# citibeth/spsparse

Hardware: AMD Instinct MI355X
Metric: nnz(C)/s for C=A*A SpGEMM (higher is better)
Workload: dtype f64

## Files before the change

### spsparse_amd/build.py

```python
import os
import subprocess
import sys
from concurrent.futures import ThreadPoolExecutor

HERE = os.path.dirname(os.path.abspath(__file__))
CSRC = os.path.join(HERE, "csrc")
VARIANT = os.environ.get("SPSAMD_VARIANT", "")
LIBDIR = os.path.join(HERE, "lib", VARIANT) if VARIANT else os.path.join(HERE, "lib")
LIB = os.path.join(LIBDIR, "libspsparse_amd.so")
SOURCES = ["prims.hip", "operand.hip", "sink.hip", "consolidate.hip", "spgemm.hip", "symbolic_heavy.hip", "k_light.hip", "k_hash.hip", "k_dense.hip", "k_tiles.hip", "k_spmm.hip", "k_add.hip", "k_stream.hip", "k_masked.hip", "k_sampled.hip", "k_select.hip", "k_extract.hip", "k_reduce.hip", "k_emult.hip", "k_solve.hip", "k_factor.hip", "k_color.hip", "k_aggregate.hip", "k_krylov.hip", "k_amg.hip",
           "workload.hip", "capi.hip", "dist.hip"]
HEADERS = ["internal.h", "devutil.h", "bank_layout.h", "spgemm_dev.h", "spgemm_host.h", "spgemm_hash.h", "workload_common.h", "x86fp.h", os.path.join("..", "..", "include", "spsparse_amd.h")]
FLAGS = ["--offload-arch=gfx950", "-O3", "-std=c++17", "-fPIC", "-ffp-contract=off",
         "-munsafe-fp-atomics", "-Wall", "-Wno-unused-result"]
FLAGS += os.environ.get("SPSAMD_CXXFLAGS", "").split()


def hipcc():
    for cand in (os.environ.get("HIPCC"), "/opt/rocm/bin/hipcc", "hipcc"):
        if cand and (os.path.isabs(cand) and os.path.exists(cand) or not os.path.isabs(cand)):
            return cand
    return "hipcc"


def _stale(target, deps):
    if not os.path.exists(target):
        return True
    t = os.path.getmtime(target)
    return any(os.path.getmtime(d) > t for d in deps)


def build(force=False, verbose=False):
    os.makedirs(LIBDIR, exist_ok=True)
    hdrs = [os.path.join(CSRC, h) for h in HEADERS]
    objs, jobs = [], []
    for s in SOURCES:
        src = os.path.join(CSRC, s)
        obj = os.path.join(LIBDIR, s.replace(".hip", ".o"))
        objs.append(obj)
        if force or _stale(obj, [src] + hdrs):
            jobs.append([hipcc()] + FLAGS + ["-c", src, "-o", obj])

    def run(cmd):
# ... 14 lines not shown
```

### spsparse_amd/csrc/capi.hip

```cpp
#include "internal.h"

#include <cstdio>
#include <cstdlib>
#include <cstring>
#include <algorithm>
#include <exception>
#include <vector>

using namespace spsamd;

#define API_GUARD(ctx, ...)                                                         \
	if ((ctx)->busy) { (ctx)->last_error = "context busy: a streamed multiply is delivering on it"; return SPSAMD_EINVAL; } \
	try { __VA_ARGS__ }                                                             \
	catch (const spsamd::Error &e) { (ctx)->last_error = e.msg; return e.code; }    \
	catch (const std::bad_alloc &) { (ctx)->last_error = "host allocation failed"; return SPSAMD_ENOMEM; } \
	catch (const std::exception &e) { (ctx)->last_error = e.what(); return SPSAMD_EINVAL; }

extern "C" const char *spsamd_version(void) { return "spsparse_amd 0.2 (gfx950)"; }

extern "C" int spsamd_ctx_create(spsamd_ctx **out, int device, void *hip_stream)
{
	if (!out) return SPSAMD_EINVAL;
	*out = nullptr;
	int ndev = 0;
	if (hipGetDeviceCount(&ndev) != hipSuccess || ndev == 0) { (void)hipGetLastError(); return SPSAMD_ENODEVICE; }
	if (device < 0) { if (hipGetDevice(&device) != hipSuccess) return SPSAMD_ENODEVICE; }
	if (device >= ndev) return SPSAMD_ENODEVICE;
	if (hipSetDevice(device) != hipSuccess) return SPSAMD_ENODEVICE;
	spsamd_ctx *c = new (std::nothrow) spsamd_ctx();
	if (!c) return SPSAMD_ENOMEM;
	c->device = device;
	hipDeviceProp_t prop;
	if (hipGetDeviceProperties(&prop, device) == hipSuccess) c->num_cu = prop.multiProcessorCount;
	if (hip_stream) { c->stream = (hipStream_t)hip_stream; c->own_stream = false; }
	else {
		if (hipStreamCreateWithFlags(&c->stream, hipStreamNonBlocking) != hipSuccess) { delete c; return SPSAMD_EHIP; }
		c->own_stream = true;
	}
	for (auto &e : c->ev) if (hipEventCreate(&e) != hipSuccess) { spsamd_ctx_destroy(c); return SPSAMD_EHIP; }
	for (auto &e : c->ev2) if (hipEventCreate(&e) != hipSuccess) { spsamd_ctx_destroy(c); return SPSAMD_EHIP; }
	if (hipStreamCreateWithFlags(&c->side, hipStreamNonBlocking) != hipSuccess) { spsamd_ctx_destroy(c); return SPSAMD_EHIP; }
	for (auto &e : c->ev_side) if (hipEventCreateWithFlags(&e, hipEventDisableTiming) != hipSuccess) { spsamd_ctx_destroy(c); return SPSAMD_EHIP; }
	if (hipStreamCreateWithFlags(&c->side2, hipStreamNonBlocking) != hipSuccess) { spsamd_ctx_destroy(c); return SPSAMD_EHIP; }
	for (auto &e : c->ev_side2) if (hipEventCreateWithFlags(&e, hipEventDisableTiming) != hipSuccess) { spsamd_ctx_destroy(c); return SPSAMD_EHIP; }
	static const char *const knobs[] = {"window", "cell_cap", "dense_min", "no_tiles", "xcd", "emit_path", "light_path", "no_wmajor", "direct_min", "tiles_v1", "long_cap", "long_dense_min", "index_budget_mb", "trace", "light_two_pass", "spmm_path", "spmm_long_min", "add_path", "masked_path", "sampled_path", "select_path", "extract_path", "reduce_path", "emult_path", "tile_walk", "solve_path", "solve_row", "solve_fuse_rows", "factor_path", "factor_row", "factor_fuse_rows", "factor_serial_work", "factor_lds_row", "color_path", "color_row", "color_fuse_rows", "color_wave_deg", "agg_path", "agg_row", "agg_fuse_rows", "agg_wave_deg", "agg_per_rows", "pcg_check_every", "pcg_fuse", "amg_path", "amg_fuse_rows"};
	static const char *const envs[] = {"SPSAMD_W", "SPSAMD_CELL_CAP", "SPSAMD_DENSE_MIN", "SPSAMD_NO_TILES", "SPSAMD_XCD", "SPSAMD_EMIT_PATH", "SPSAMD_LIGHT_PATH", "SPSAMD_NO_WMAJOR", "SPSAMD_DIRECT_MIN", "SPSAMD_TILES_V1", "SPSAMD_LONG_CAP", "SPSAMD_LONG_DENSE_MIN", "SPSAMD_INDEX_BUDGET_MB", "SPSAMD_TRACE", "SPSAMD_LIGHT_TWO_PASS", "SPSAMD_SPMM_PATH", "SPSAMD_SPMM_LONG_MIN", "SPSAMD_ADD_PATH", "SPSAMD_MASKED_PATH", "SPSAMD_SAMPLED_PATH", "SPSAMD_SELECT_PATH", "SPSAMD_EXTRACT_PATH", "SPSAMD_REDUCE_PATH", "SPSAMD_EMULT_PATH", "SPSAMD_TILE_WALK", "SPSAMD_SOLVE_PATH", "SPSAMD_SOLVE_ROW", "SPSAMD_SOLVE_FUSE_ROWS", "SPSAMD_FACTOR_PATH", "SPSAMD_FACTOR_ROW", "SPSAMD_FACTOR_FUSE_ROWS", "SPSAMD_FACTOR_SERIAL_WORK", "SPSAMD_FACTOR_LDS_ROW", "SPSAMD_COLOR_PATH", "SPSAMD_COLOR_ROW", "SPSAMD_COLOR_FUSE_ROWS", "SPSAMD_COLOR_WAVE_DEG", "SPSAMD_AGG_PATH", "SPSAMD_AGG_ROW", "SPSAMD_AGG_FUSE_ROWS", "SPSAMD_AGG_WAVE_DEG", "SPSAMD_AGG_PER_ROWS", "SPSAMD_PCG_CHECK_EVERY", "SPSAMD_PCG_FUSE", "SPSAMD_AMG_PATH", "SPSAMD_AMG_FUSE_ROWS"};
	static_assert(sizeof knobs / sizeof knobs[0] == sizeof envs / sizeof envs[0], "one environment variable per knob");
	for (size_t k = 0; k < sizeof knobs / sizeof knobs[0]; ++k)
		if (const char *e = getenv(envs[k])) (void)spsamd_ctx_set_tuning(c, knobs[k], atol(e));
#ifdef SPSAMD_ABLATIONS
	if (const char *e = getenv("SPSAMD_DBG")) c->tune.dbg = atoi(e);
#endif
	*out = c;
	return SPSAMD_OK;
}

extern "C" int spsamd_ctx_set_tuning(spsamd_ctx *c, const char *name, long value)
{
	if (!c || !name) return SPSAMD_EINVAL;
	if (c->busy) { c->last_error = "context busy: a streamed multiply is delivering on it"; return SPSAMD_EINVAL; }
	struct { const char *n; int *p; } tab[] = {
		{"window", &c->tune.window}, {"cell_cap", &c->tune.cell_cap}, {"dense_min", &c->tune.dense_min},
		{"no_tiles", &c->tune.no_tiles}, {"xcd", &c->tune.xcd}, {"emit_path", &c->tune.emit_path},
		{"light_path", &c->tune.light_path}, {"no_wmajor", &c->tune.no_wmajor}, {"direct_min", &c->tune.direct_min}, {"tiles_v1", &c->tune.tiles_v1}, {"long_cap", &c->tune.long_cap}, {"long_dense_min", &c->tune.long_dense_min}, {"index_budget_mb", &c->tune.index_budget_mb}, {"trace", &c->tune.trace}, {"light_two_pass", &c->tune.light_two_pass},
		{"spmm_path", &c->tune.spmm_path}, {"spmm_long_min", &c->tune.spmm_long_min}, {"add_path", &c->tune.add_path},
		{"masked_path", &c->tune.masked_path}, {"sampled_path", &c->tune.sampled_path}, {"select_path", &c->tune.select_path},
		{"extract_path", &c->tune.extract_path}, {"reduce_path", &c->tune.reduce_path}, {"emult_path", &c->tune.emult_path},
		{"tile_walk", &c->tune.tile_walk}, {"solve_path", &c->tune.solve_path}, {"solve_row", &c->tune.solve_row},
		{"solve_fuse_rows", &c->tune.solve_fuse_rows}, {"factor_path", &c->tune.factor_path}, {"factor_row", &c->tune.factor_row},
		{"factor_fuse_rows", &c->tune.factor_fuse_rows}, {"factor_serial_work", &c->tune.factor_serial_work},
		{"factor_lds_row", &c->tune.factor_lds_row}, {"color_path", &c->tune.color_path}, {"color_row", &c->tune.color_row},
		{"color_fuse_rows", &c->tune.color_fuse_rows}, {"color_wave_deg", &c->tune.color_wave_deg},
		{"agg_path", &c->tune.agg_path}, {"agg_row", &c->tune.agg_row}, {"agg_fuse_rows", &c->tune.agg_fuse_rows},
		{"agg_wave_deg", &c->tune.agg_wave_deg}, {"agg_per_rows", &c->tune.agg_per_rows},
		{"pcg_check_every", &c->tune.pcg_check_every}, {"pcg_fuse", &c->tune.pcg_fuse},
		{"amg_path", &c->tune.amg_path}, {"amg_fuse_rows", &c->tune.amg_fuse_rows},
	};
	for (auto &t : tab) if (!std::strcmp(t.n, name)) { *t.p = (int)value; return SPSAMD_OK; }
	c->last_error = std::string("unknown tuning knob: ") + name;
	return SPSAMD_EINVAL;
}

extern "C" void spsamd_ctx_destroy(spsamd_ctx *c)
{
	if (!c) return;
	(void)hipSetDevice(c->device);
	if (c->stream) (void)hipStreamSynchronize(c->stream);
	if (c->side) (void)hipStreamSynchronize(c->side);
	if (c->side2) (void)hipStreamSynchronize(c->side2);
	c->arena.release();
	c->out[0].release(); c->out[1].release();
	c->rowstat_n.release(); c->rowstat_s.release(); c->rowstat_h.release();
	if (c->pinned) (void)hipHostFree(c->pinned);
	if (c->stream_pinned) (void)hipHostFree(c->stream_pinned);
	for (auto &e : c->ev) if (e) (void)hipEventDestroy(e);
	for (auto &e : c->ev2) if (e) (void)hipEventDestroy(e);
	for (auto &e : c->ev_side) if (e) (void)hipEventDestroy(e);
// ... 573 lines not shown
```

### spsparse_amd/csrc/internal.h

```cpp
#pragma once

#include <hip/hip_runtime.h>
#include <stdint.h>
#include <stddef.h>
#include <string>
#include <vector>

#include "../../include/spsparse_amd.h"

namespace spsamd {


struct Error {
	int code;
	std::string msg;
};

#define SPS_HIP(call)                                                              \
	do {                                                                           \
		hipError_t e_ = (call);                                                    \
		if (e_ != hipSuccess)                                                      \
			throw ::spsamd::Error{SPSAMD_EHIP, std::string(#call) + ": " + hipGetErrorString(e_)}; \
	} while (0)

// ... 13 lines not shown
	void reset();
	void release();
	void reserve(size_t bytes);
	template <class T> T *get(size_t n) { return (T *)alloc(n * sizeof(T)); }
};

struct DevBuf {
	void *p = nullptr;
	size_t cap = 0;
	void ensure(size_t bytes);
	void release();
	bool holds(const void *q) const { return p && q && (const char *)q >= (const char *)p && (const char *)q < (const char *)p + cap; }
};

struct OutSet {
	DevBuf i, j, v;
	bool holds(const void *q) const { return i.holds(q) || j.holds(q) || v.holds(q); }
	void release() { i.release(); j.release(); v.release(); }
};

struct Tuning {
	int window = 0;
	int cell_cap = 0;
	int dense_min = 0;
	int no_tiles = 0;
	int xcd = 2;
	int emit_path = 0;
	int light_path = 0;
	int light_two_pass = 0;
	int no_wmajor = 0;
	int tiles_v1 = 0;
	int long_cap = 0;
	int long_dense_min = 0;
	int direct_min = 0;
	int trace = 0;
	int index_budget_mb = 0;
	int spmm_path = 0;
	int spmm_long_min = 0;
	int add_path = 0;
	int masked_path = 0;
	int sampled_path = 0;
	int select_path = 0;
	int extract_path = 0;
	int reduce_path = 0;
	int tile_walk = 0;
	int emult_path = 0;
	int solve_path = 0;
	int solve_row = 0;
	int solve_fuse_rows = 0;
	int factor_path = 0;
	int factor_row = 0;
	int factor_fuse_rows = 0;
	int factor_serial_work = 0;
	int factor_lds_row = 0;
	int color_path = 0;
	int color_row = 0;
	int color_fuse_rows = 0;
	int color_wave_deg = 0;
	int agg_path = 0;
	int agg_row = 0;
	int agg_fuse_rows = 0;
	int agg_wave_deg = 0;
	int agg_per_rows = 0;
	int pcg_check_every = 0;
	int pcg_fuse = 0;
	int amg_path = 0;
// ... 448 lines not shown
```

### spsparse_amd/csrc/spgemm.hip

```cpp
#include "spgemm_host.h"

namespace spsamd {

__global__ void k_pack_b(const int32_t *bcol, const double *bval, uint32_t n, BTup *out)
{
	uint32_t i = blockIdx.x * blockDim.x + threadIdx.x;
	if (i >= n) return;
	double v = bval[i];
	BTup t; t.col = bcol[i]; t.vlo = (uint32_t)__double2loint(v); t.vhi = (uint32_t)__double2hiint(v);
	out[i] = t;
}


__global__ void k_elem_len(const int32_t *acol, const uint32_t *bptr, uint32_t n, uint32_t *lo, uint32_t *len)
{
	uint32_t e = blockIdx.x * blockDim.x + threadIdx.x;
	if (e < n) { int32_t k = acol[e]; uint32_t b = bptr[k]; lo[e] = b; len[e] = bptr[k + 1] - b; }
}

__global__ void k_apply_scalej(const int32_t *acol, const double *aval, uint32_t n, const int32_t *pos, const double *sval,
	int32_t ninner, int32_t *acol2, double *aval2)
{
	uint32_t e = blockIdx.x * blockDim.x + threadIdx.x;
	if (e >= n) return;
	int32_t k = acol[e];
	int32_t q = pos[k];
	if (q < 0) { acol2[e] = ninner; aval2[e] = 0.0; }
	else { acol2[e] = k; aval2[e] = aval[e] * sval[q]; }
}

struct BinCounters { unsigned long long rows[NBIN]; unsigned long long prods[NBIN]; unsigned long long tuples[NBIN]; unsigned long long too_big; };

__device__ __forceinline__ int bin_of(uint32_t P)
{
	if (P == 0) return 0;
	if (P <= 8) return 1;
	if (P <= 16) return 2;
	if (P <= 32) return 3;
	if (P <= 64) return 4;
	if (P <= 512) return 5;
	if (P <= 2048) return 6;
	if (P <= MID_MAX) return 7;
	return 8;
}

constexpr int CLS_ITEMS = 4;

__global__ __launch_bounds__(256) void k_classify(const uint32_t *beg, const int32_t *id, uint32_t nrows, const int64_t *pref, const uint32_t *elen,
	const int32_t *si_pos, const double *si_val, uint32_t *rprod, uint8_t *rbin, BinCounters *bc)
{
	__shared__ unsigned int s_rows[NBIN];
	__shared__ unsigned long long s_prods[NBIN];
	__shared__ unsigned long long s_tuples[NBIN];
	if (threadIdx.x < NBIN) { s_rows[threadIdx.x] = 0; s_prods[threadIdx.x] = 0; s_tuples[threadIdx.x] = 0; }
	__syncthreads();
	for (int it = 0; it < CLS_ITEMS; ++it) {
		uint32_t r = (blockIdx.x * CLS_ITEMS + it) * 256u + threadIdx.x;
		int b = -1;
		uint32_t P = 0, La = 0;
		if (r < nrows) {
			const uint32_t b0 = beg[r], b1 = beg[r + 1];
			La = b1 - b0;
			if (La <= 8) {
				for (uint32_t e = b0; e < b1; ++e) P += elen[e];
			} else {
				const int64_t d = pref[b1] - pref[b0];
				if (d > 0xFFFFFFFFll) atomicAdd(&bc->too_big, 1ull);
				P = (uint32_t)d;
			}
			if (si_pos) {
				int32_t q = si_pos[id[r]];
				if (q < 0 || si_val[q] == 0) P = 0;
			}
			b = bin_of(P);
			rprod[r] = P;
			rbin[r] = (uint8_t)b;
		}
		uint64_t todo = __ballot(b >= 0);
		while (todo) {
			int leader = __ffsll((unsigned long long)todo) - 1;
			int bb = __shfl(b, leader, 64);
			uint64_t mine = __ballot(b == bb);
			unsigned long long p = wave_reduce_sum((unsigned long long)(b == bb ? P : 0u));
			unsigned long long t = wave_reduce_sum((unsigned long long)(b == bb ? La : 0u));
			if ((int)lane_id() == leader) {
				atomicAdd(&s_rows[bb], (unsigned int)__popcll(mine));
				atomicAdd(&s_prods[bb], p);
				atomicAdd(&s_tuples[bb], t);
			}
			todo &= ~mine;
		}
	}
	__syncthreads();
	if (threadIdx.x < NBIN && s_rows[threadIdx.x]) {
		atomicAdd(&bc->rows[threadIdx.x], (unsigned long long)s_rows[threadIdx.x]);
		atomicAdd(&bc->prods[threadIdx.x], s_prods[threadIdx.x]);
		atomicAdd(&bc->tuples[threadIdx.x], s_tuples[threadIdx.x]);
	}
}

struct BinOffsets { uint32_t off[NBIN + 1]; };

__global__ __launch_bounds__(256) void k_bin_scatter(const uint8_t *rbin, uint32_t nrows, BinOffsets bo, uint32_t *cursor, uint32_t *binrows)
{
	__shared__ unsigned int s_cnt[NBIN];
	__shared__ unsigned int s_base[NBIN];
	if (threadIdx.x < NBIN) s_cnt[threadIdx.x] = 0;
// ... 306 lines not shown
static BTup *ensure_btup(spsamd_ctx *c, MultiplyArgs &a, Prepared *p)
{
	if (p->btup) return p->btup;
	wait_b_tuples(c, a);
	p->btup = p->get<BTup>((size_t)p->m.nnz + DENSE_R);
	k_pack_b<<<dim3(grid_for(p->m.nnz)), dim3(256), 0, c->stream>>>(p->m.col, p->m.val, p->m.nnz, p->btup);
	SPS_LAUNCH_CHECK();
	return p->btup;
}

BTup *prepared_btup(spsamd_ctx *c, Prepared *p)
{
	MultiplyArgs a;
	a.b_ready = nullptr;
	return ensure_btup(c, a, p);
}

struct RowClasses { Bins bins; uint32_t *rprod, *elo, *elen; BinCounters hbc; };

static RowClasses classify_rows(spsamd_ctx *c, const MultiplyArgs &a, const RowList &rl, const int32_t *acol, const uint32_t *bptr)
{
	hipStream_t st = c->stream;
	const uint32_t nnz = a.A.nnz;
	RowClasses rc;
	rc.elen = c->arena.get<uint32_t>(nnz);
	rc.elo = c->arena.get<uint32_t>(nnz);
	int64_t *pref = c->arena.get<int64_t>((size_t)nnz + 1);
	k_elem_len<<<dim3(grid_for(nnz)), dim3(256), 0, st>>>(acol, bptr, nnz, rc.elo, rc.elen);
	SPS_LAUNCH_CHECK();
	scan_exclusive_u32_i64(c, rc.elen, pref, nnz);
	rc.rprod = c->arena.get<uint32_t>(rl.nrows);
	uint8_t *rbin = c->arena.get<uint8_t>(rl.nrows);
	BinCounters *bc = get_zeroed<BinCounters>(c, 1);
	k_classify<<<dim3(grid_for(rl.nrows, 256 * CLS_ITEMS)), dim3(256), 0, st>>>(rl.beg, rl.id, rl.nrows, pref, rc.elen,
		a.si.present ? a.si.pos : nullptr, a.si.val, rc.rprod, rbin, bc);
	SPS_LAUNCH_CHECK();
	rc.hbc = read_back(c, bc);
	if (rc.hbc.too_big) throw Error{SPSAMD_EINVAL, "an output row with more than 2^32-1 scalar products is not supported"};
	Bins &bins = rc.bins;
	BinOffsets bo; uint32_t run = 0;
	for (int b = 0; b < NBIN; ++b) {
		bins.count[b] = b == 0 ? 0 : (uint32_t)rc.hbc.rows[b];
		bins.off[b] = bo.off[b] = run;
		run += bins.count[b];
	}
	bins.off[NBIN] = bo.off[NBIN] = run;
	int whole_bin = 0;
	for (int b = 1; b <= 4; ++b) if (bins.count[b] == rl.nrows) whole_bin = b;
	bins.rows = nullptr;
	if (!whole_bin) {
		bins.rows = c->arena.get<uint32_t>(run ? run : 1);
		uint32_t *cursor = get_zeroed<uint32_t>(c, NBIN);
		k_bin_scatter<<<dim3(grid_for(rl.nrows, 256 * CLS_ITEMS)), dim3(256), 0, st>>>(rbin, rl.nrows, bo, cursor, bins.rows);
		SPS_LAUNCH_CHECK();
	}
	return rc;
}

static void fill_class_counters(spsamd_result *res, const BinCounters &h)
{
	const struct { int first, last; uint64_t *rows, *prods, *tuples; } cls[3] = {{1, 4, &res->rows_light, &res->products_light, &res->tuples_light},
		{5, 7, &res->rows_mid, &res->products_mid, &res->tuples_mid}, {8, 8, &res->rows_heavy, &res->products_heavy, &res->tuples_heavy}};
	res->products = 0;
	for (auto &k : cls) {
		*k.rows = *k.prods = *k.tuples = 0;
		for (int b = k.first; b <= k.last; ++b) { *k.rows += h.rows[b]; *k.prods += h.prods[b]; *k.tuples += h.tuples[b]; }
		res->products += *k.prods;
	}
}

static int64_t build_segments(spsamd_ctx *c, const MultiplyArgs &a, const RowList &rl, const RowClasses &rc, const RowMeta &m, Prepared *pb,
	Heavy &hv, MidCells &mc, SinkParams &sk, spsamd_result *res)
{
	const Bins &bins = rc.bins;
	uint32_t *nseg = c->arena.get<uint32_t>(rl.nrows);
	fill_u32(c, nseg, 1u, rl.nrows);
	hv.n = bins.count[8]; hv.tuples = rc.hbc.tuples[8]; hv.coo = a.sink_kind == SPSAMD_SINK_COO;
	if (hv.n) heavy_prepare(c, hv, bins, m, a.B, m.bptr, SENTINEL_ROWS, nseg, (a.sink_flags & SPSAMD_SINK_ORDERED) != 0, (a.sink_flags & SPSAMD_SINK_EXACT_PATTERN) != 0, pb);
	if (a.static_walk) hv.tile_ctr = nullptr;
	uint32_t *segbase = nullptr; int64_t nsegs = 0;
	if (hv.coo) {
		int64_t *segbase64 = c->arena.get<int64_t>((size_t)rl.nrows + 1);
		scan_exclusive_u32_i64(c, nseg, segbase64, rl.nrows);
		nsegs = read_back(c, segbase64 + rl.nrows);
		if (nsegs >= (int64_t(1) << 32)) throw Error{SPSAMD_EINVAL, "too many output segments"};
		segbase = c->arena.get<uint32_t>((size_t)rl.nrows + 1);
		scan_exclusive_u32_u32(c, nseg, segbase, rl.nrows);
	}
	if (hv.n) heavy_cells(c, hv, m, segbase);
	for (int k = 0; k < 3; ++k) {
		uint32_t nb = bins.count[5 + k];
		if (!nb) continue;
		mc.cells[k] = c->arena.get<Cell>(nb);
		k_row_cells<<<dim3(grid_for(nb)), dim3(256), 0, c->stream>>>(bins.rows + bins.off[5 + k], nb, rl.beg, rl.id, rc.rprod, segbase, mc.cells[k]);
		SPS_LAUNCH_CHECK();
	}
	res->cells_hash = (uint64_t)hv.ncell[0] + hv.ncell[1] + hv.ncell[2] + hv.ncell[3] + hv.ntcell + hv.ntcell2;
	res->cells_dense = hv.ncell[CLS_DENSE]; res->window = hv.n ? (uint32_t)hv.W : 0u;
	res->products_dense = hv.clsprod[CLS_DENSE]; res->products_tiles = hv.clsprod[NCLS]; res->products_direct = hv.clsprod[NCLS + 1];
	sk.segbase = segbase;
	return nsegs;
}

struct Work { const Bins &bins; const MidCells &mc; Heavy &hv; const RowMeta &m; const EmitParams &ep; };

template <int MODE>
static void launch_pass(spsamd_ctx *c, const Work &w, const SinkParams &sk, const int (&mark)[5])
{
	auto record = [&](int e) { if (e != EV_NONE) SPS_HIP(hipEventRecord(c->ev[e], c->stream)); };
	record(mark[0]);
	launch_light<MODE>(c, w.bins, w.m, w.ep, sk);
	record(mark[1]);
	launch_mid<MODE>(c, w.bins, w.mc, w.m, w.ep, sk);
	record(mark[2]);
	if (MODE != MODE_STORE && w.hv.n) heavy_sort_lists(c, w.hv);
	launch_heavy_hash<MODE>(c, w.hv, w.m, w.ep, sk);
	record(mark[3]);
	c->join_side(true, true);
	launch_heavy_dense<MODE>(c, w.hv, w.m, w.ep, sk);
	record(mark[4]);
}

static void numeric_digest(spsamd_ctx *c, const MultiplyArgs &a, const Work &w, SinkParams &sk, spsamd_result *res)
{
	DigestSlot *slots = digest_begin(c, a, a.A.nrow, sk, res);
	launch_pass<MODE_DIGEST>(c, w, sk, {EV_N0, EV_N1, EV_N2, EV_N3, EV_N4});
	check_kernel_error(digest_end(c, slots, sk.err, res));
	res->ms_light = elapsed(c->ev[EV_N0], c->ev[EV_N1]); res->ms_mid = elapsed(c->ev[EV_N1], c->ev[EV_N2]);
	res->ms_heavy = elapsed(c->ev[EV_N2], c->ev[EV_N4]); res->ms_dense = elapsed(c->ev[EV_N3], c->ev[EV_N4]);
}

static uint64_t close_holes(spsamd_ctx *c, const SinkParams &sk, int64_t nsegs, int64_t reserved)
{
	hipStream_t st = c->stream;
	struct HolesErr { unsigned long long holes, err; };
	unsigned long long *holes = get_zeroed<unsigned long long>(c, 2);
	k_seg_holes<<<dim3(grid_for((size_t)nsegs)), dim3(256), 0, st>>>(sk.segcount, sk.segactual, (uint32_t)nsegs, holes, sk.err);
	SPS_LAUNCH_CHECK();
	const HolesErr he = read_back(c, (const HolesErr *)holes);
	check_kernel_error(he.err);
	const uint64_t nnz = (uint64_t)reserved - he.holes;
	if (he.holes) {
		int64_t *newoff = c->arena.get<int64_t>((size_t)nsegs + 1);
		scan_exclusive_u32_i64(c, sk.segactual, newoff, (size_t)nsegs);
		int32_t *ti = c->arena.get<int32_t>(nnz ? nnz : 1), *tj = c->arena.get<int32_t>(nnz ? nnz : 1);
		double *tv = c->arena.get<double>(nnz ? nnz : 1);
// ... 218 lines not shown
```

### spsparse_amd/csrc/spgemm_dev.h

```cpp
#pragma once
#include "internal.h"
#include "devutil.h"

#include <algorithm>
#include <type_traits>
#include <cstdio>
#include <cstdlib>
#include <vector>

namespace spsamd {

enum { MODE_COUNT = 0, MODE_STORE = 1, MODE_DIGEST = 2 };

constexpr int NBIN = 9;
#ifndef MID_MAX_V
#define MID_MAX_V 4096
#endif
constexpr uint32_t MID_MAX = MID_MAX_V;
#ifndef DENSE_U
#define DENSE_U 1
#endif
#ifndef HASH_U
#define HASH_U 4
#endif
constexpr int DIGEST_SLOTS = 1024;

struct EmitParams {
	double C;
	const int32_t *si_pos; const double *si_val;
	const int32_t *sk_pos; const double *sk_val;
	int emit_path;
#ifdef SPSAMD_ABLATIONS
	int dbg;
#endif
	uint32_t wshift;
	uint32_t ncolbits;
	int ordered;
	int pattern;
};

#ifdef SPSAMD_ABLATIONS
#define ABL(ep, bit) ((ep).dbg & (bit))
static __device__ int g_abl;
#define ABLG(bit) (g_abl & (bit))
#else
#define ABL(ep, bit) false
#define ABLG(bit) false
// ... 667 lines not shown
```

### spsparse_amd/csrc/spgemm_host.h

```cpp
#pragma once
#include "spgemm_dev.h"

namespace spsamd {

struct Bins {
	uint32_t count[NBIN];
	uint32_t off[NBIN + 1];
	uint32_t *rows;
};

struct MidCells { Cell *cells[3] = {nullptr, nullptr, nullptr}; };

struct TooWide { uint64_t width; };
constexpr uint64_t COLBLK = (uint64_t)2048 << 14;

struct Heavy {
	uint32_t n = 0;
	uint64_t tuples = 0;
	uint32_t *rows = nullptr;
	uint32_t *bwin = nullptr;
	uint32_t *bocc = nullptr;
	uint32_t nbw = 0;
	uint32_t nwin = 0, nwin1 = 0;
	uint32_t *winprod = nullptr;
	uint32_t ncell[NCLS] = {};
	Cell *cells[NCLS] = {};
	CellBases cnt{}, base{};
	uint32_t *xb[NCLS] = {};
	int W = 8192;
	uint32_t cell_cap = CELL_CAP_DEFAULT, dense_min = DENSE_MIN_DEFAULT;
	TileBases tb{};
	uint32_t ntile = 0, ntcell = 0;
	TileBases tb2{};
	uint32_t ntile2 = 0, ntcell2 = 0;
	uint32_t direct_min = 0;
	int tiles2 = 0;
	uint32_t *tile_ctr = nullptr;
	uint32_t span_cap = 0;
	uint32_t alt_cap = 0, alt_span = 0;
	unsigned long long *alt_cells = nullptr;
	uint32_t long_cap = 0, long_dense_min = 0;
	bool coo = false;
	unsigned long long clsprod[NCLS + 2] = {};
	uint32_t *wptr = nullptr;
// ... 37 lines not shown
	SinkParams sk2 = sk;
	sk2.stamps = c->arena.get<unsigned long long>((size_t)grid * STAMP_COLS);
	fill_zero(c, sk2.stamps, (size_t)grid * STAMP_COLS * sizeof(unsigned long long));
	return sk2;
}
static inline void stamps_report(spsamd_ctx *c, const SinkParams &sk2, unsigned grid, const char *kernel, const char *const *nm, int ncol, int nmax = 0)
{
	std::vector<unsigned long long> h((size_t)grid * STAMP_COLS);
	SPS_HIP(hipMemcpyAsync(h.data(), sk2.stamps, h.size() * 8, hipMemcpyDeviceToHost, c->stream));
	SPS_HIP(hipStreamSynchronize(c->stream));
	double sum[STAMP_COLS] = {}, mx = 0;
	for (unsigned g = 0; g < grid; ++g) {
		double t = 0;
		for (int i = 0; i < STAMP_COLS; ++i) { sum[i] += (double)h[(size_t)g * STAMP_COLS + i]; if (i < nmax) t += (double)h[(size_t)g * STAMP_COLS + i]; }
		mx = std::max(mx, t);
	}
	fprintf(stderr, "%s stamps (mean cycles per workgroup, grid %u", kernel, grid);
	if (nmax) fprintf(stderr, "; max total %.3g", mx);
	fprintf(stderr, "):");
	for (int i = 0; i < ncol; ++i) fprintf(stderr, " %s %.4g", nm[i], sum[i] / grid);
	fprintf(stderr, "\n");
}
#else
static inline const SinkParams &stamps_sink(spsamd_ctx *, const SinkParams &sk, unsigned) { return sk; }
static inline void stamps_report(spsamd_ctx *, const SinkParams &, unsigned, const char *, const char *const *, int, int = 0) { }
#endif

template <int MODE> void launch_light(spsamd_ctx *c, const Bins &b, const RowMeta &m, const EmitParams &ep, const SinkParams &sk);
template <int MODE> void launch_light_direct_s(spsamd_ctx *c, uint32_t maxp, uint32_t nrow, const uint32_t *aptr, const int32_t *acol, const double *aval,
	const uint32_t *bptr, const ConMat &B, bool k64, const EmitParams &ep, const SinkParams &sk, unsigned long long *pc);
void launch_light_gather(spsamd_ctx *c, uint32_t nrow, uint32_t S, const uint32_t *cnt, const int64_t *off,
	const int32_t *si, const int32_t *sj, const double *sv, int32_t *oi, int32_t *oj, double *ov);
template <int MODE> void launch_mid(spsamd_ctx *c, const Bins &b, const MidCells &mc, const RowMeta &m, const EmitParams &ep, const SinkParams &sk);
template <int MODE> void launch_hash_windowed(spsamd_ctx *c, const Heavy &hv, const RowMeta &m, const EmitParams &ep, const SinkParams &sk);
template <int MODE> void launch_tiles_v1(spsamd_ctx *c, const Heavy &hv, const RowMeta &m, const EmitParams &ep, const SinkParams &sk);
template <int MODE> void launch_tiles_bm(spsamd_ctx *c, const Heavy &hv, const RowMeta &m, const EmitParams &ep, const SinkParams &sk);
template <int MODE> void launch_tiles_hash2(spsamd_ctx *c, const Heavy &hv, const RowMeta &m, const EmitParams &ep, const SinkParams &sk);
template <int MODE> void launch_tiles_direct(spsamd_ctx *c, const Heavy &hv, const RowMeta &m, const EmitParams &ep, const SinkParams &sk);
template <int MODE> void launch_heavy_dense(spsamd_ctx *c, const Heavy &hv, const RowMeta &m0, const EmitParams &ep, const SinkParams &sk);

int heavy_b_index(spsamd_ctx *c, const ConMat &B, const uint32_t *bptr, uint32_t extra, uint64_t nheavy, Prepared *pb);
void heavy_prepare(spsamd_ctx *c, Heavy &hv, const Bins &bins, const RowMeta &m, const ConMat &B, const uint32_t *bptr,
	uint32_t extra, uint32_t *nseg, bool ordered, bool pattern, Prepared *pb);
void heavy_cells(spsamd_ctx *c, Heavy &hv, const RowMeta &m, const uint32_t *segbase);
void heavy_sort_lists(spsamd_ctx *c, Heavy &hv);

void spgemm_once(spsamd_ctx *c, MultiplyArgs &a, spsamd_result *res);

#ifdef SPSAMD_ABLATIONS
void set_ablation_word(spsamd_ctx *c, int word);
#endif

#define SPSAMD_INSTANTIATE_MODES(decl_macro) decl_macro(MODE_COUNT) decl_macro(MODE_STORE) decl_macro(MODE_DIGEST)

}
```

Measured before the change: 165.4 billion.

## Add specialized hash kernel for mid-size rows with few A entries

Introduces new bins and a k_few kernel for mid-class output rows whose A row has at most a few nonzeros (default 8). Each block loads the short list of A segments into lanes, maps each product index straight to its B tuple with readlane-based prefix lookup, and prefetches the next cells in a software pipeline. This removes per-segment iteration overhead of the generic mid kernel for such rows. It applies only to arrival-order sinks, and it adds three more kernel launches plus a larger bin table.

```diff
diff --git a/spsparse_amd/build.py b/spsparse_amd/build.py
--- a/spsparse_amd/build.py
+++ b/spsparse_amd/build.py
@@ -8,7 +8,7 @@
 VARIANT = os.environ.get("SPSAMD_VARIANT", "")
 LIBDIR = os.path.join(HERE, "lib", VARIANT) if VARIANT else os.path.join(HERE, "lib")
 LIB = os.path.join(LIBDIR, "libspsparse_amd.so")
-SOURCES = ["prims.hip", "operand.hip", "sink.hip", "consolidate.hip", "spgemm.hip", "symbolic_heavy.hip", "k_light.hip", "k_hash.hip", "k_dense.hip", "k_tiles.hip", "k_spmm.hip", "k_add.hip", "k_stream.hip", "k_masked.hip", "k_sampled.hip", "k_select.hip", "k_extract.hip", "k_reduce.hip", "k_emult.hip", "k_solve.hip", "k_factor.hip", "k_color.hip", "k_aggregate.hip", "k_krylov.hip", "k_amg.hip",
+SOURCES = ["prims.hip", "operand.hip", "sink.hip", "consolidate.hip", "spgemm.hip", "symbolic_heavy.hip", "k_light.hip", "k_hash.hip", "k_few.hip", "k_dense.hip", "k_tiles.hip", "k_spmm.hip", "k_add.hip", "k_stream.hip", "k_masked.hip", "k_sampled.hip", "k_select.hip", "k_extract.hip", "k_reduce.hip", "k_emult.hip", "k_solve.hip", "k_factor.hip", "k_color.hip", "k_aggregate.hip", "k_krylov.hip", "k_amg.hip",
            "workload.hip", "capi.hip", "dist.hip"]
 HEADERS = ["internal.h", "devutil.h", "bank_layout.h", "spgemm_dev.h", "spgemm_host.h", "spgemm_hash.h", "workload_common.h", "x86fp.h", os.path.join("..", "..", "include", "spsparse_amd.h")]
 FLAGS = ["--offload-arch=gfx950", "-O3", "-std=c++17", "-fPIC", "-ffp-contract=off",
diff --git a/spsparse_amd/csrc/capi.hip b/spsparse_amd/csrc/capi.hip
--- a/spsparse_amd/csrc/capi.hip
+++ b/spsparse_amd/csrc/capi.hip
@@ -43,8 +43,8 @@
 	for (auto &e : c->ev_side) if (hipEventCreateWithFlags(&e, hipEventDisableTiming) != hipSuccess) { spsamd_ctx_destroy(c); return SPSAMD_EHIP; }
 	if (hipStreamCreateWithFlags(&c->side2, hipStreamNonBlocking) != hipSuccess) { spsamd_ctx_destroy(c); return SPSAMD_EHIP; }
 	for (auto &e : c->ev_side2) if (hipEventCreateWithFlags(&e, hipEventDisableTiming) != hipSuccess) { spsamd_ctx_destroy(c); return SPSAMD_EHIP; }
-	static const char *const knobs[] = {"window", "cell_cap", "dense_min", "no_tiles", "xcd", "emit_path", "light_path", "no_wmajor", "direct_min", "tiles_v1", "long_cap", "long_dense_min", "index_budget_mb", "trace", "light_two_pass", "spmm_path", "spmm_long_min", "add_path", "masked_path", "sampled_path", "select_path", "extract_path", "reduce_path", "emult_path", "tile_walk", "solve_path", "solve_row", "solve_fuse_rows", "factor_path", "factor_row", "factor_fuse_rows", "factor_serial_work", "factor_lds_row", "color_path", "color_row", "color_fuse_rows", "color_wave_deg", "agg_path", "agg_row", "agg_fuse_rows", "agg_wave_deg", "agg_per_rows", "pcg_check_every", "pcg_fuse", "amg_path", "amg_fuse_rows"};
-	static const char *const envs[] = {"SPSAMD_W", "SPSAMD_CELL_CAP", "SPSAMD_DENSE_MIN", "SPSAMD_NO_TILES", "SPSAMD_XCD", "SPSAMD_EMIT_PATH", "SPSAMD_LIGHT_PATH", "SPSAMD_NO_WMAJOR", "SPSAMD_DIRECT_MIN", "SPSAMD_TILES_V1", "SPSAMD_LONG_CAP", "SPSAMD_LONG_DENSE_MIN", "SPSAMD_INDEX_BUDGET_MB", "SPSAMD_TRACE", "SPSAMD_LIGHT_TWO_PASS", "SPSAMD_SPMM_PATH", "SPSAMD_SPMM_LONG_MIN", "SPSAMD_ADD_PATH", "SPSAMD_MASKED_PATH", "SPSAMD_SAMPLED_PATH", "SPSAMD_SELECT_PATH", "SPSAMD_EXTRACT_PATH", "SPSAMD_REDUCE_PATH", "SPSAMD_EMULT_PATH", "SPSAMD_TILE_WALK", "SPSAMD_SOLVE_PATH", "SPSAMD_SOLVE_ROW", "SPSAMD_SOLVE_FUSE_ROWS", "SPSAMD_FACTOR_PATH", "SPSAMD_FACTOR_ROW", "SPSAMD_FACTOR_FUSE_ROWS", "SPSAMD_FACTOR_SERIAL_WORK", "SPSAMD_FACTOR_LDS_ROW", "SPSAMD_COLOR_PATH", "SPSAMD_COLOR_ROW", "SPSAMD_COLOR_FUSE_ROWS", "SPSAMD_COLOR_WAVE_DEG", "SPSAMD_AGG_PATH", "SPSAMD_AGG_ROW", "SPSAMD_AGG_FUSE_ROWS", "SPSAMD_AGG_WAVE_DEG", "SPSAMD_AGG_PER_ROWS", "SPSAMD_PCG_CHECK_EVERY", "SPSAMD_PCG_FUSE", "SPSAMD_AMG_PATH", "SPSAMD_AMG_FUSE_ROWS"};
+	static const char *const knobs[] = {"window", "cell_cap", "dense_min", "no_tiles", "xcd", "emit_path", "light_path", "no_wmajor", "direct_min", "tiles_v1", "long_cap", "long_dense_min", "few_max", "index_budget_mb", "trace", "light_two_pass", "spmm_path", "spmm_long_min", "add_path", "masked_path", "sampled_path", "select_path", "extract_path", "reduce_path", "emult_path", "tile_walk", "solve_path", "solve_row", "solve_fuse_rows", "factor_path", "factor_row", "factor_fuse_rows", "factor_serial_work", "factor_lds_row", "color_path", "color_row", "color_fuse_rows", "color_wave_deg", "agg_path", "agg_row", "agg_fuse_rows", "agg_wave_deg", "agg_per_rows", "pcg_check_every", "pcg_fuse", "amg_path", "amg_fuse_rows"};
+	static const char *const envs[] = {"SPSAMD_W", "SPSAMD_CELL_CAP", "SPSAMD_DENSE_MIN", "SPSAMD_NO_TILES", "SPSAMD_XCD", "SPSAMD_EMIT_PATH", "SPSAMD_LIGHT_PATH", "SPSAMD_NO_WMAJOR", "SPSAMD_DIRECT_MIN", "SPSAMD_TILES_V1", "SPSAMD_LONG_CAP", "SPSAMD_LONG_DENSE_MIN", "SPSAMD_FEW_MAX", "SPSAMD_INDEX_BUDGET_MB", "SPSAMD_TRACE", "SPSAMD_LIGHT_TWO_PASS", "SPSAMD_SPMM_PATH", "SPSAMD_SPMM_LONG_MIN", "SPSAMD_ADD_PATH", "SPSAMD_MASKED_PATH", "SPSAMD_SAMPLED_PATH", "SPSAMD_SELECT_PATH", "SPSAMD_EXTRACT_PATH", "SPSAMD_REDUCE_PATH", "SPSAMD_EMULT_PATH", "SPSAMD_TILE_WALK", "SPSAMD_SOLVE_PATH", "SPSAMD_SOLVE_ROW", "SPSAMD_SOLVE_FUSE_ROWS", "SPSAMD_FACTOR_PATH", "SPSAMD_FACTOR_ROW", "SPSAMD_FACTOR_FUSE_ROWS", "SPSAMD_FACTOR_SERIAL_WORK", "SPSAMD_FACTOR_LDS_ROW", "SPSAMD_COLOR_PATH", "SPSAMD_COLOR_ROW", "SPSAMD_COLOR_FUSE_ROWS", "SPSAMD_COLOR_WAVE_DEG", "SPSAMD_AGG_PATH", "SPSAMD_AGG_ROW", "SPSAMD_AGG_FUSE_ROWS", "SPSAMD_AGG_WAVE_DEG", "SPSAMD_AGG_PER_ROWS", "SPSAMD_PCG_CHECK_EVERY", "SPSAMD_PCG_FUSE", "SPSAMD_AMG_PATH", "SPSAMD_AMG_FUSE_ROWS"};
 	static_assert(sizeof knobs / sizeof knobs[0] == sizeof envs / sizeof envs[0], "one environment variable per knob");
 	for (size_t k = 0; k < sizeof knobs / sizeof knobs[0]; ++k)
 		if (const char *e = getenv(envs[k])) (void)spsamd_ctx_set_tuning(c, knobs[k], atol(e));
@@ -62,7 +62,7 @@
 	struct { const char *n; int *p; } tab[] = {
 		{"window", &c->tune.window}, {"cell_cap", &c->tune.cell_cap}, {"dense_min", &c->tune.dense_min},
 		{"no_tiles", &c->tune.no_tiles}, {"xcd", &c->tune.xcd}, {"emit_path", &c->tune.emit_path},
-		{"light_path", &c->tune.light_path}, {"no_wmajor", &c->tune.no_wmajor}, {"direct_min", &c->tune.direct_min}, {"tiles_v1", &c->tune.tiles_v1}, {"long_cap", &c->tune.long_cap}, {"long_dense_min", &c->tune.long_dense_min}, {"index_budget_mb", &c->tune.index_budget_mb}, {"trace", &c->tune.trace}, {"light_two_pass", &c->tune.light_two_pass},
+		{"light_path", &c->tune.light_path}, {"no_wmajor", &c->tune.no_wmajor}, {"direct_min", &c->tune.direct_min}, {"tiles_v1", &c->tune.tiles_v1}, {"long_cap", &c->tune.long_cap}, {"long_dense_min", &c->tune.long_dense_min}, {"few_max", &c->tune.few_max}, {"index_budget_mb", &c->tune.index_budget_mb}, {"trace", &c->tune.trace}, {"light_two_pass", &c->tune.light_two_pass},
 		{"spmm_path", &c->tune.spmm_path}, {"spmm_long_min", &c->tune.spmm_long_min}, {"add_path", &c->tune.add_path},
 		{"masked_path", &c->tune.masked_path}, {"sampled_path", &c->tune.sampled_path}, {"select_path", &c->tune.select_path},
 		{"extract_path", &c->tune.extract_path}, {"reduce_path", &c->tune.reduce_path}, {"emult_path", &c->tune.emult_path},
diff --git a/spsparse_amd/csrc/internal.h b/spsparse_amd/csrc/internal.h
--- a/spsparse_amd/csrc/internal.h
+++ b/spsparse_amd/csrc/internal.h
@@ -69,6 +69,7 @@
 	int tiles_v1 = 0;
 	int long_cap = 0;
 	int long_dense_min = 0;
+	int few_max = 0;
 	int direct_min = 0;
 	int trace = 0;
 	int index_budget_mb = 0;
diff --git a/spsparse_amd/csrc/k_few.hip b/spsparse_amd/csrc/k_few.hip
--- /dev/null
+++ b/spsparse_amd/csrc/k_few.hip
@@ -0,0 +1,157 @@
+#include "spgemm_host.h"
+#include "spgemm_hash.h"
+
+namespace spsamd {
+
+struct FewSegs { uint32_t lo, len; double a; };
+
+__device__ __forceinline__ FewSegs few_segs_load(const RowMeta &m, uint32_t beg, uint32_t end)
+{
+	const uint32_t e = beg + (lane_id() & (FEW_LMAX - 1u));
+	const bool act = lane_id() < FEW_LMAX && e < end;
+	const uint32_t ec = act ? e : beg;
+	FewSegs s;
+	s.lo = m.elo[ec];
+	const uint32_t len = m.elen[ec];
+	s.a = m.aval[ec];
+	s.len = act ? len : 0u;
+	return s;
+}
+
+template <int U> struct FewB { BTup t[U]; double a[U]; uint32_t prods; };
+
+template <int U, int NT>
+__device__ __forceinline__ void few_request(FewB<U> &b, const RowMeta &m, const FewSegs &s, const Cell &rec, uint32_t cap)
+{
+	const uint32_t inc = wave_inclusive_scan_u32(s.len);
+	const uint32_t La = min(rec.end - rec.beg, FEW_LMAX);
+	uint32_t prods = (uint32_t)__builtin_amdgcn_readlane((int)inc, 63);
+	if (rec.prods > cap || rec.end - rec.beg > FEW_LMAX) prods = 0;
+	const uint32_t pref = inc - s.len;
+	uint32_t p[U], off[U];
+#pragma unroll
+	for (int u = 0; u < U; ++u) {
+		const uint32_t q = (uint32_t)u * NT + threadIdx.x;
+		p[u] = q < prods ? q : 0u;
+		off[u] = 0u; b.a[u] = 0.0;
+	}
+	for (uint32_t g = 0; g < La; ++g) {
+		const uint32_t ps = (uint32_t)__builtin_amdgcn_readlane((int)pref, (int)g);
+		const uint32_t rel = (uint32_t)__builtin_amdgcn_readlane((int)s.lo, (int)g) - ps;
+		const double as = __hiloint2double(__builtin_amdgcn_readlane(__double2hiint(s.a), (int)g), __builtin_amdgcn_readlane(__double2loint(s.a), (int)g));
+#pragma unroll
+		for (int u = 0; u < U; ++u) {
+			const bool in = ps <= p[u];
+			off[u] = in ? rel : off[u];
+			b.a[u] = in ? as : b.a[u];
+		}
+	}
+#pragma unroll
+	for (int u = 0; u < U; ++u) b.t[u] = m.btup[off[u] + p[u]];
+	b.prods = prods;
+}
+
+template <int T, int NT, int MODE>
+__global__ __launch_bounds__(NT) void k_few(const Cell *cells, uint32_t ncell, RowMeta m, EmitParams ep, SinkParams sk)
+{
+	constexpr int U = (T / 2 + NT - 1) / NT;
+	__shared__ int32_t h_key[T];
+	__shared__ double h_val[MODE == MODE_COUNT ? 1 : T];
+	__shared__ uint16_t occ[T / 2];
+	__shared__ uint64_t s_sort[MODE == MODE_STORE ? T / 2 : 1];
+	__shared__ uint16_t s_cnt[MODE == MODE_STORE ? 16 * ((T / 2 + NT - 1) / NT) * (NT / 64) : 1];
+	__shared__ uint32_t scr32[NT / 64 + 1];
+	__shared__ uint32_t s_nocc[2];
+	__shared__ unsigned long long s_u64[2 * (NT / 64)];
+	__shared__ double s_f64[NT / 64];
+
+	const unsigned tid = threadIdx.x, lane = lane_id();
+	for (int q = tid; q < T; q += NT) { h_key[q] = -1; if (MODE != MODE_COUNT) h_val[q] = 0.0; }
+	if (tid < 2) s_nocc[tid] = 0;
+	__syncthreads();
+	DigestAcc dacc{0, 0, 0.0};
+	uint32_t oflip = 0;
+
+	const uint32_t stride = gridDim.x, first = blockIdx.x, clast = ncell - 1u;
+	const uint32_t zlane = cell_pend_zero();
+	Cell rec0 = cells[min(first, clast)], rec1 = cells[min(first + stride, clast)], rec2 = cells[min(first + 2u * stride, clast)];
+	CellPend pend3 = cell_pend_load(cells, min(first + 3u * stride, clast), zlane);
+	FewSegs seg1 = few_segs_load(m, rec1.beg, rec1.end), seg2 = few_segs_load(m, rec2.beg, rec2.end);
+	FewB<U> b0;
+	few_request<U, NT>(b0, m, few_segs_load(m, rec0.beg, rec0.end), rec0, (uint32_t)(T / 2));
+	for (uint32_t ci = first; ci < ncell; ci += stride) {
+		const Cell cell = rec0;
+		if ((cell.prods > (uint32_t)(T / 2) || cell.end - cell.beg > FEW_LMAX) && tid == 0) atomicOr(sk.err, 1u);
+		FewB<U> b1;
+		few_request<U, NT>(b1, m, seg1, rec1, (uint32_t)(T / 2));
+		rec0 = rec1; rec1 = rec2; seg1 = seg2;
+		rec2 = cell_from_pend(pend3);
+		seg2 = few_segs_load(m, rec2.beg, rec2.end);
+		pend3 = cell_pend_load(cells, min(ci + 4u * stride, clast), zlane);
+
+		{
+			uint32_t slot_of[U]; uint64_t newmask[U]; uint32_t nnew = 0;
+#pragma unroll
+			for (int u = 0; u < U; ++u) {
+				bool isnew = false;
+				uint32_t h = 0;
+				if ((uint32_t)u * NT + tid < b0.prods) {
+					const int32_t col = b0.t[u].col;
+					h = hash_slot<T>(col);
+					for (;;) {
+						int32_t old = atomicCAS(&h_key[h], -1, col);
+						if (old == -1) { isnew = true; break; }
+						if (old == col) break;
+						if constexpr ((T & (T - 1)) == 0) h = (h + 1) & (T - 1);
+						else h = h + 1 == (uint32_t)T ? 0u : h + 1;
+					}
+					if (MODE != MODE_COUNT) atomicAdd(&h_val[h], b0.a[u] * btup_val(b0.t[u]));
+				}
+				slot_of[u] = h;
+				newmask[u] = __ballot(isnew);
+				nnew += (uint32_t)__popcll(newmask[u]);
+			}
+			if (nnew) {
+				uint32_t base = 0;
+				if (lane == 0) base = lds_add_rtn_u32(&s_nocc[oflip], nnew);
+				base = (uint32_t)__builtin_amdgcn_readfirstlane((int)base);
+#pragma unroll
+				for (int u = 0; u < U; ++u) {
+					if ((newmask[u] >> lane) & 1ull) occ[base + __popcll(newmask[u] & lanemask_lt())] = (uint16_t)slot_of[u];
+					base += (uint32_t)__popcll(newmask[u]);
+				}
+			}
+		}
+		lds_barrier();
+		const uint32_t nocc = s_nocc[oflip];
+		if (tid == 0) s_nocc[oflip ^ 1u] = 0;
+		oflip ^= 1u;
+		hash_emit<T, NT, MODE, false>(nocc, cell.rowid, cell.seg, ep, sk, h_key, h_val, occ, s_sort, scr32, dacc, s_cnt, 0, ep.ncolbits, m, cell.beg, cell.end, -1.0);
+		lds_barrier();
+		b0 = b1;
+	}
+	if (MODE == MODE_DIGEST) digest_flush<NT>(sk.digest, dacc.cnt, dacc.hash, dacc.sum, s_u64, s_f64);
+}
+
+template <int T, int NT, int MODE>
+static void launch_few(spsamd_ctx *c, const Cell *cells, uint32_t ncell, const RowMeta &m, const EmitParams &ep, const SinkParams &sk)
+{
+	if (!ncell) return;
+	const unsigned grid = std::min<unsigned>(ncell, (unsigned)(c->num_cu * resident_per_cu<&k_few<T, NT, MODE>>(NT)));
+	k_few<T, NT, MODE><<<dim3(grid), dim3(NT), 0, c->stream>>>(cells, ncell, m, ep, sk);
+	SPS_LAUNCH_CHECK();
+}
+
+template <int MODE>
+void launch_mid_few(spsamd_ctx *c, const Bins &b, const MidCells &mc, const RowMeta &m, const EmitParams &ep, const SinkParams &sk)
+{
+	launch_few<1024, 256, MODE>(c, mc.few[0], b.count[BIN_FEW], m, ep, sk);
+	launch_few<4096, 512, MODE>(c, mc.few[1], b.count[BIN_FEW + 1], m, ep, sk);
+	launch_few<8192, 1024, MODE>(c, mc.few[2], b.count[BIN_FEW + 2], m, ep, sk);
+}
+
+template void launch_mid_few<MODE_COUNT>(spsamd_ctx *, const Bins &, const MidCells &, const RowMeta &, const EmitParams &, const SinkParams &);
+template void launch_mid_few<MODE_STORE>(spsamd_ctx *, const Bins &, const MidCells &, const RowMeta &, const EmitParams &, const SinkParams &);
+template void launch_mid_few<MODE_DIGEST>(spsamd_ctx *, const Bins &, const MidCells &, const RowMeta &, const EmitParams &, const SinkParams &);
+
+}
diff --git a/spsparse_amd/csrc/spgemm.hip b/spsparse_amd/csrc/spgemm.hip
--- a/spsparse_amd/csrc/spgemm.hip
+++ b/spsparse_amd/csrc/spgemm.hip
@@ -47,7 +47,7 @@
 constexpr int CLS_ITEMS = 4;
 
 __global__ __launch_bounds__(256) void k_classify(const uint32_t *beg, const int32_t *id, uint32_t nrows, const int64_t *pref, const uint32_t *elen,
-	const int32_t *si_pos, const double *si_val, uint32_t *rprod, uint8_t *rbin, BinCounters *bc)
+	const int32_t *si_pos, const double *si_val, int few_max, uint32_t *rprod, uint8_t *rbin, BinCounters *bc)
 {
 	__shared__ unsigned int s_rows[NBIN];
 	__shared__ unsigned long long s_prods[NBIN];
@@ -73,6 +73,7 @@
 				if (q < 0 || si_val[q] == 0) P = 0;
 			}
 			b = bin_of(P);
+			if (b >= 5 && b <= 7 && (int)La <= few_max) b += BIN_FEW - 5;
 			rprod[r] = P;
 			rbin[r] = (uint8_t)b;
 		}
@@ -445,8 +446,10 @@
 	rc.rprod = c->arena.get<uint32_t>(rl.nrows);
 	uint8_t *rbin = c->arena.get<uint8_t>(rl.nrows);
 	BinCounters *bc = get_zeroed<BinCounters>(c, 1);
+	const bool arrival = !(a.sink_flags & (SPSAMD_SINK_ORDERED | SPSAMD_SINK_EXACT_PATTERN));
+	const int few_max = !arrival || c->tune.few_max < 0 ? -1 : (c->tune.few_max == 0 ? FEW_MAX_DEFAULT : std::min(c->tune.few_max, (int)FEW_LMAX));
 	k_classify<<<dim3(grid_for(rl.nrows, 256 * CLS_ITEMS)), dim3(256), 0, st>>>(rl.beg, rl.id, rl.nrows, pref, rc.elen,
-		a.si.present ? a.si.pos : nullptr, a.si.val, rc.rprod, rbin, bc);
+		a.si.present ? a.si.pos : nullptr, a.si.val, few_max, rc.rprod, rbin, bc);
 	SPS_LAUNCH_CHECK();
 	rc.hbc = read_back(c, bc);
 	if (rc.hbc.too_big) throw Error{SPSAMD_EINVAL, "an output row with more than 2^32-1 scalar products is not supported"};
@@ -472,14 +475,14 @@
 
 static void fill_class_counters(spsamd_result *res, const BinCounters &h)
 {
-	const struct { int first, last; uint64_t *rows, *prods, *tuples; } cls[3] = {{1, 4, &res->rows_light, &res->products_light, &res->tuples_light},
-		{5, 7, &res->rows_mid, &res->products_mid, &res->tuples_mid}, {8, 8, &res->rows_heavy, &res->products_heavy, &res->tuples_heavy}};
+	const struct { int first, last; uint64_t *rows, *prods, *tuples; } cls[4] = {{1, 4, &res->rows_light, &res->products_light, &res->tuples_light},
+		{5, 7, &res->rows_mid, &res->products_mid, &res->tuples_mid}, {8, 8, &res->rows_heavy, &res->products_heavy, &res->tuples_heavy},
+		{BIN_FEW, BIN_FEW + 2, &res->rows_mid, &res->products_mid, &res->tuples_mid}};
 	res->products = 0;
-	for (auto &k : cls) {
-		*k.rows = *k.prods = *k.tuples = 0;
-		for (int b = k.first; b <= k.last; ++b) { *k.rows += h.rows[b]; *k.prods += h.prods[b]; *k.tuples += h.tuples[b]; }
-		res->products += *k.prods;
-	}
+	res->rows_light = res->products_light = res->tuples_light = res->rows_mid = res->products_mid = res->tuples_mid = 0;
+	res->rows_heavy = res->products_heavy = res->tuples_heavy = 0;
+	for (auto &k : cls)
+		for (int b = k.first; b <= k.last; ++b) { *k.rows += h.rows[b]; *k.prods += h.prods[b]; *k.tuples += h.tuples[b]; res->products += h.prods[b]; }
 }
 
 static int64_t build_segments(spsamd_ctx *c, const MultiplyArgs &a, const RowList &rl, const RowClasses &rc, const RowMeta &m, Prepared *pb,
@@ -501,13 +504,16 @@
 		scan_exclusive_u32_u32(c, nseg, segbase, rl.nrows);
 	}
 	if (hv.n) heavy_cells(c, hv, m, segbase);
-	for (int k = 0; k < 3; ++k) {
-		uint32_t nb = bins.count[5 + k];
+	for (int k = 0; k < 6; ++k) {
+		const int bin = k < 3 ? 5 + k : BIN_FEW + k - 3;
+		uint32_t nb = bins.count[bin];
 		if (!nb) continue;
-		mc.cells[k] = c->arena.get<Cell>(nb);
-		k_row_cells<<<dim3(grid_for(nb)), dim3(256), 0, c->stream>>>(bins.rows + bins.off[5 + k], nb, rl.beg, rl.id, rc.rprod, segbase, mc.cells[k]);
+		Cell *&list = k < 3 ? mc.cells[k] : mc.few[k - 3];
+		list = c->arena.get<Cell>(nb);
+		k_row_cells<<<dim3(grid_for(nb)), dim3(256), 0, c->stream>>>(bins.rows + bins.off[bin], nb, rl.beg, rl.id, rc.rprod, segbase, list);
 		SPS_LAUNCH_CHECK();
 	}
+	if (c->tune.trace) fprintf(stderr, "few cells: mid %u\n", bins.count[BIN_FEW] + bins.count[BIN_FEW + 1] + bins.count[BIN_FEW + 2]);
 	res->cells_hash = (uint64_t)hv.ncell[0] + hv.ncell[1] + hv.ncell[2] + hv.ncell[3] + hv.ntcell + hv.ntcell2;
 	res->cells_dense = hv.ncell[CLS_DENSE]; res->window = hv.n ? (uint32_t)hv.W : 0u;
 	res->products_dense = hv.clsprod[CLS_DENSE]; res->products_tiles = hv.clsprod[NCLS]; res->products_direct = hv.clsprod[NCLS + 1];
@@ -525,6 +531,7 @@
 	launch_light<MODE>(c, w.bins, w.m, w.ep, sk);
 	record(mark[1]);
 	launch_mid<MODE>(c, w.bins, w.mc, w.m, w.ep, sk);
+	launch_mid_few<MODE>(c, w.bins, w.mc, w.m, w.ep, sk);
 	record(mark[2]);
 	if (MODE != MODE_STORE && w.hv.n) heavy_sort_lists(c, w.hv);
 	launch_heavy_hash<MODE>(c, w.hv, w.m, w.ep, sk);
diff --git a/spsparse_amd/csrc/spgemm_dev.h b/spsparse_amd/csrc/spgemm_dev.h
--- a/spsparse_amd/csrc/spgemm_dev.h
+++ b/spsparse_amd/csrc/spgemm_dev.h
@@ -12,7 +12,10 @@
 
 enum { MODE_COUNT = 0, MODE_STORE = 1, MODE_DIGEST = 2 };
 
-constexpr int NBIN = 9;
+constexpr int NBIN = 12;
+constexpr int BIN_FEW = 9;
+constexpr uint32_t FEW_LMAX = 16;
+constexpr int FEW_MAX_DEFAULT = 8;
 #ifndef MID_MAX_V
 #define MID_MAX_V 4096
 #endif
diff --git a/spsparse_amd/csrc/spgemm_host.h b/spsparse_amd/csrc/spgemm_host.h
--- a/spsparse_amd/csrc/spgemm_host.h
+++ b/spsparse_amd/csrc/spgemm_host.h
@@ -9,7 +9,7 @@
 	uint32_t *rows;
 };
 
-struct MidCells { Cell *cells[3] = {nullptr, nullptr, nullptr}; };
+struct MidCells { Cell *cells[3] = {nullptr, nullptr, nullptr}; Cell *few[3] = {nullptr, nullptr, nullptr}; };
 
 struct TooWide { uint64_t width; };
 constexpr uint64_t COLBLK = (uint64_t)2048 << 14;
@@ -113,6 +113,7 @@
 void launch_light_gather(spsamd_ctx *c, uint32_t nrow, uint32_t S, const uint32_t *cnt, const int64_t *off,
 	const int32_t *si, const int32_t *sj, const double *sv, int32_t *oi, int32_t *oj, double *ov);
 template <int MODE> void launch_mid(spsamd_ctx *c, const Bins &b, const MidCells &mc, const RowMeta &m, const EmitParams &ep, const SinkParams &sk);
+template <int MODE> void launch_mid_few(spsamd_ctx *c, const Bins &b, const MidCells &mc, const RowMeta &m, const EmitParams &ep, const SinkParams &sk);
 template <int MODE> void launch_hash_windowed(spsamd_ctx *c, const Heavy &hv, const RowMeta &m, const EmitParams &ep, const SinkParams &sk);
 template <int MODE> void launch_tiles_v1(spsamd_ctx *c, const Heavy &hv, const RowMeta &m, const EmitParams &ep, const SinkParams &sk);
 template <int MODE> void launch_tiles_bm(spsamd_ctx *c, const Heavy &hv, const RowMeta &m, const EmitParams &ep, const SinkParams &sk);
```

Measured after the change: 167.6 billion, median of 6. 1.01x the previous value.
